# Corv/CUDA-GMM-MPI

Measured on NVIDIA H100. Metric: EM iterations/sec at N=10M D=24 K=64; E-step HBM GB/s vs roofline, higher is better.
Workload: dtype f32

## Files before the change

cuda-gmm-mpi_b200/csrc/kernels_tc.cu:

```cuda
#include <cuda.h>
#include <cudaTypedefs.h>
#include <cuda_fp16.h>
#if defined(__F16C__) && defined(__AVX__)
#include <immintrin.h>
#endif
#include <cuda_runtime.h>

#include <cmath>
#include <cstdio>
#include <cstdlib>
#include <cstring>
#include <string>
#include <type_traits>
#include <vector>

#include "host_math.h"
#include "kernels_tc.cuh"
#include "mstep_rows.h"
#include "tc_ptx.cuh"

namespace gmm {

using namespace ptx;

// ... 269 lines not shown
        auto add_to_racc = [&](float (&acc)[HPC][NCL / 2]) {
#pragma unroll
            for (int c = 0; c < 2; c++) {
#pragma unroll
                for (int j = 0; j < 16; j++) {
                    const int q = 16 * c + j;
                    racc[q * C::NCT] += acc[q / (NCL / 2)][q % (NCL / 2)];
                }
                asm volatile("" ::: "memory");
            }
        };
        uint32_t fh[2][2][4], fl[2][2][4];
        float2 za[4];
        int held = -1;
        auto group = [&](int i, auto hc, uint32_t (&gh)[2][4], uint32_t (&gl)[2][4]) {
            constexpr int h = decltype(hc)::value;
            const int rs = i % kNRAW, rph = (i / kNRAW) & 1;
            const int os = i % kNST, oph = (i / kNST) & 1;
            const uint32_t zst = zs0 + rs * C::RAWX;
            const uint32_t gam = smem_u32(smem + C::OFF_G + os * C::G_STAGE);
            const bool new1 = chain_starts(i, mt), new2 = chain2_starts(i, mt);
            if constexpr (h == 0) {
                mbar_wait_parked(&raw_full[rs], rph, 100);
                load_row(zst + fa, za);
            }
            float2 zb0[4], zb1[4];
            load_row(zst + fb[2 * h], zb0);
            load_row(zst + fb[2 * h + 1], zb1);
            build_half(za, zb0, zb1, mg[2 * h], mg[2 * h + 1], gh, gl);
            if constexpr (h == 0) mbar_wait_parked(&op_full[os], oph, 100);
            wgmma_fence();
            issue_half<NCL>(ex[h], rm[h], gh, gl, gam, new1, new2);
            wgmma_commit();
            if constexpr (h == HPC - 1) {
                __syncwarp();
                if (lane == 0) mbar_arrive(&raw_empty[rs]);
            }
            wgmma_wait<1>();
            if constexpr (h == 0) {
                __syncwarp();
                if (lane == 0 && held >= 0) mbar_arrive(&op_empty[held]);
            }
            if constexpr (h == HPC - 1) {
                held = os;
                if (chain_ends(i, mt, nsub)) {
                    wgmma_wait<0>();
                    __syncwarp();
                    if (lane == 0) mbar_arrive(&op_empty[os]);
                    held = -1;
#if GMM_MSTEP_CUT != 3
                    add_to_racc(ex);
                    if (chain2_ends(i, mt, nsub)) add_to_racc(rm);
#endif
                }
            }
        };
        using H0 = std::integral_constant<int, 0>;
        using H1 = std::integral_constant<int, 1>;
        if constexpr (HPC == 2) {
            for (int i = 0; i < nsub; i++) {
                group(i, H0{}, fh[0], fl[0]);
                group(i, H1{}, fh[1], fl[1]);
            }
        } else {
            int i = 0;
            for (; i + 1 < nsub; i += 2) {
                group(i, H0{}, fh[0], fl[0]);
                group(i + 1, H0{}, fh[1], fl[1]);
            }
            if (i < nsub) group(i, H0{}, fh[0], fl[0]);
        }
        wgmma_wait<0>();
#if GMM_MSTEP_CUT == 3
#pragma unroll
        for (int h = 0; h < HPC; h++)
#pragma unroll
            for (int j = 0; j < NCL / 2; j++) ex[h][j] += rm[h][j];
        add_to_racc(ex);
#endif
        const int nranges = gridDim.x * HPC / 2;
#pragma unroll
        for (int h = 0; h < HPC; h++)
#pragma unroll
            for (int j = 0; j < NCL / 2; j += 2) {
                const int q = h * (NCL / 2) + j;
                const int row = ((hx & 1) + h) * 64 + wq * 16 + gid + 8 * ((j >> 1) & 1);
                const int col = (j >> 2) * 8 + 2 * qd;
                const int ty = blockIdx.y * (NCL / kNCL) + col / kNCL;
                float* dst = scratch + ((((size_t)ty * nranges + range) * C::MT + mt) * 128 + row) * kNCL + col % kNCL;
                *reinterpret_cast<float2*>(dst) = make_float2(racc[q * C::NCT], racc[(q + 1) * C::NCT]);
            }
    }
}

__global__ void standardise_soa_kernel(const float* __restrict__ xs, float* __restrict__ zs, size_t pitch, int n, int D,
                                       const float* __restrict__ shift_f, const float* __restrict__ inv_scale_f) {
    const int d = blockIdx.y;
    const float s = shift_f[d], isc = inv_scale_f[d];
    const float* x = xs + (size_t)d * pitch;
    float* z = zs + (size_t)d * pitch;
    for (long long e = (long long)blockIdx.x * blockDim.x + threadIdx.x; e < n; e += (long long)gridDim.x * blockDim.x)
        z[e] = __fmul_rn(__fsub_rn(x[e], s), isc);
}

__global__ void __launch_bounds__(256)
mstep_tc_finalize_kernel(const float* __restrict__ scratch, int ncta_x, int MT, int K, int F, const int3* __restrict__ rowmap,
                         const double* __restrict__ scale, double* __restrict__ stats, double wscale) {
    constexpr int NQ = 256 / kNCL;
    __shared__ double part[NQ][kNCL];
    const int3 rm = rowmap[blockIdx.x];
    if (rm.x < 0) return;
    const int mt = blockIdx.x / 128, row = blockIdx.x % 128;
    const int col = threadIdx.x & (kNCL - 1), q = threadIdx.x / kNCL;
    double fac = wscale / (double)kGammaScale;
    if (rm.y >= 0) fac *= scale[rm.y];
    if (rm.z >= 0) fac *= scale[rm.z];
    for (int ty = 0; ty * kNCL < K; ty++) {
        double s = 0;
        for (int cx = q; cx < ncta_x; cx += NQ)
            s += (double)scratch[(((size_t)(ty * ncta_x + cx) * MT + mt) * 128 + row) * kNCL + col];
        part[q][col] = s;
        __syncthreads();
        const int k = ty * kNCL + col;
        if (q == 0 && k < K) {
            double t = 0;
#pragma unroll
            for (int u = 0; u < NQ; u++) t += part[u][col];
            stats[(size_t)k * F + rm.x] += t * fac;
        }
        __syncthreads();
    }
}


template <int D> struct ECfg {
    static_assert(D % 8 == 0, "tensor E-step: D must be a multiple of 8");
    static constexpr int CP = D / 8;
    static constexpr int NLO = (CP + 1 + 1) / 2 * 2;
    static constexpr int NCHKB = CP + NLO;
    static constexpr int GB = 16;
    static constexpr int N = GB * 8;
    static constexpr int MAXSG = 64 / GB;
    static constexpr int B_BLOCK = NCHKB * N * 16;
    static constexpr int B_SG = CP * B_BLOCK;
    static constexpr int OFF_B = 0;
    static constexpr int OFF_CK = OFF_B + MAXSG * B_SG;
    static constexpr int OFF_SH = OFF_CK + 512;
    static constexpr int OFF_BAR = OFF_SH + 256;
    static constexpr int SMEM_BYTES = OFF_BAR + 64;
    static constexpr int NWG = 2;
    static constexpr int THREADS = 128 * NWG;
};

#ifndef GMM_ESTEP_CUT
#define GMM_ESTEP_CUT 0
#endif

template <int D>
__device__ __forceinline__ void tc_stage_operand(uint8_t* smem, const uint8_t* __restrict__ b_img, const float* __restrict__ ck,
                                                 const float* __restrict__ shift_f, const float* __restrict__ inv_scale_f, int NSG) {
    using C = ECfg<D>;
    uint64_t* b_full = reinterpret_cast<uint64_t*>(smem + C::OFF_BAR);
    float* ck_s = reinterpret_cast<float*>(smem + C::OFF_CK);
    float* sh_s = reinterpret_cast<float*>(smem + C::OFF_SH);
    if (threadIdx.x == 0) { mbar_init(b_full, 1); fence_mbar_init(); }
    if (threadIdx.x < 64) { ck_s[threadIdx.x] = ck[threadIdx.x] * 1.4426950408889634f; ck_s[64 + threadIdx.x] = ck[64 + threadIdx.x]; }
    if (threadIdx.x < D) { sh_s[threadIdx.x] = shift_f[threadIdx.x]; sh_s[32 + threadIdx.x] = inv_scale_f[threadIdx.x]; }
    __syncthreads();
    if (threadIdx.x == 0) {
        mbar_arrive_expect_tx(b_full, (uint32_t)NSG * C::B_SG);
        for (int g = 0; g < NSG * C::CP; g++) tma_load_1d(smem + C::OFF_B + g * C::B_BLOCK, b_img + (size_t)g * C::B_BLOCK, C::B_BLOCK, b_full);
    }
}

template <int D>
__device__ __forceinline__ void tc_split_rows(const float2 (&xa)[D / 8], const float2 (&xb)[D / 8], const float* sh_s, const float* isc_s,
                                              int qd, uint32_t (&zh)[D / 8][2], uint32_t (&zl)[D / 8][2]) {
#pragma unroll
    for (int j = 0; j < D / 8; j++) {
        const float s0 = sh_s[8 * j + 2 * qd], s1 = sh_s[8 * j + 2 * qd + 1];
        const float i0 = isc_s[8 * j + 2 * qd], i1 = isc_s[8 * j + 2 * qd + 1];
#pragma unroll
        for (int r = 0; r < 2; r++) {
            const float2 x = r ? xb[j] : xa[j];
            const float z0 = __fmul_rn(__fsub_rn(x.x, s0), i0), z1 = __fmul_rn(__fsub_rn(x.y, s1), i1);
            const __half2 h = __floats2half2_rn(z0, z1);
            const float2 f = __half22float2(h);
            zh[j][r] = *reinterpret_cast<const uint32_t*>(&h);
            zl[j][r] = pack_half2(z0 - f.x, z1 - f.y);
        }
    }
}

template <int D>
__device__ __forceinline__ void tc_issue_group(float (&acc)[32], const uint32_t (&zh)[D / 8][2], const uint32_t (&zl)[D / 8][2],
                                               uint32_t bsg, int c, int h, uint32_t ones) {
    using C = ECfg<D>;
    constexpr int CP = C::CP;
    constexpr uint32_t CH = C::N * 16;
    const uint32_t bb = bsg + (uint32_t)c * C::B_BLOCK + (uint32_t)h * (CH / 2);
    wgmma_fence();
#pragma unroll
    for (int j = c; j < CP; j++)
        wgmma_m64n64k16_rs(acc, zh[j][0], zh[j][1], zh[j][0], zh[j][1], make_smem_desc(bb + j * CH, CP * CH, 128), j > c);
#pragma unroll
    for (int p = c; p < CP + 1; p += 2) {
        const int x = p, y = p + 1;
        if (y <= CP) {
            const uint32_t yc = y < CP ? (uint32_t)y : 2u * CP;
            const uint32_t a2 = y < CP ? zl[y < CP ? y : 0][0] : ones, a3 = y < CP ? zl[y < CP ? y : 0][1] : ones;
            wgmma_m64n64k16_rs(acc, zl[x][0], zl[x][1], a2, a3, make_smem_desc(bb + x * CH, (yc - x) * CH, 128), true);
        } else {
            wgmma_m64n64k16_rs(acc, 0u, 0u, ones, ones, make_smem_desc(bb + c * CH, (2 * CP - c) * CH, 128), true);
        }
    }
}

template <int D, int NSG>
__device__ __forceinline__ void tc_tile_logits(const uint32_t (&zh)[D / 8][2], const uint32_t (&zl)[D / 8][2], uint32_t bsm,
                                               const float* ck_s, int qd, uint32_t ones, float (&lg)[ECfg<D>::MAXSG][8]) {
    using C = ECfg<D>;
    constexpr int CP = C::CP;
    float acc[2][32];
    tc_issue_group<D>(acc[0], zh, zl, bsm, 0, 0, ones);
    wgmma_commit();
#pragma unroll
    for (int sg = 0; sg < C::MAXSG; sg++) {
        if (sg >= NSG) {
#pragma unroll
            for (int u = 0; u < 8; u++) lg[sg][u] = -INFINITY;
            continue;
        }
        const uint32_t bsg = bsm + (uint32_t)sg * C::B_SG;
        float sq[32];
#pragma unroll
        for (int u = 0; u < 32; u++) sq[u] = 0.f;
#pragma unroll
        for (int c = 0; c < CP; c++) {
#pragma unroll
            for (int h = 0; h < 2; h++) {
                if (sg + 1 == NSG && c + 1 == CP && h == 1) {
                    wgmma_wait<0>();
                } else {
                    if (h == 0) tc_issue_group<D>(acc[1], zh, zl, bsg, c, 1, ones);
                    else if (c + 1 < CP) tc_issue_group<D>(acc[0], zh, zl, bsg, c + 1, 0, ones);
                    else tc_issue_group<D>(acc[0], zh, zl, bsg + C::B_SG, 0, 0, ones);
                    wgmma_commit();
                    wgmma_wait<1>();
                }
                wgmma_pin(acc[h]);
                const float(&a)[32] = acc[h];
#if GMM_ESTEP_CUT == 1
                sq[0] += a[0];
#else
#pragma unroll
                for (int i = 0; i < 8; i++) {
                    float& s0 = sq[16 * h + 2 * i];
                    float& s1 = sq[16 * h + 2 * i + 1];
                    s0 = fmaf(a[4 * i], a[4 * i], fmaf(a[4 * i + 1], a[4 * i + 1], s0));
                    s1 = fmaf(a[4 * i + 2], a[4 * i + 2], fmaf(a[4 * i + 3], a[4 * i + 3], s1));
                }
#endif
            }
        }
#if GMM_ESTEP_CUT == 1
        for (int u = 0; u < 8; u++) lg[sg][u] = sq[0];
        continue;
#endif
        float w[16];
        const bool b1 = qd & 1, b2 = (qd >> 1) & 1;
#pragma unroll
        for (int u = 0; u < 16; u++) {
            const float send = b1 ? sq[u] : sq[16 + u], keep = b1 ? sq[16 + u] : sq[u];
            w[u] = keep + __shfl_xor_sync(0xffffffffu, send, 1);
        }
#pragma unroll
        for (int u = 0; u < 8; u++) {
            const float send = b2 ? w[u] : w[8 + u], keep = b2 ? w[8 + u] : w[u];
            const float qv = keep + __shfl_xor_sync(0xffffffffu, send, 2);
            const int k = sg * C::GB + 8 * (qd & 1) + 4 * (qd >> 1) + (u >> 1);
            lg[sg][u] = fmaf(ck_s[64 + k], qv, ck_s[k]);
        }
    }
}

template <int D, int NSG, bool WT = false>
__global__ void __launch_bounds__(ECfg<D>::THREADS, 1)
estep_tc_kernel(const float* __restrict__ x_aos, const uint8_t* __restrict__ b_img, const float* __restrict__ ck,
                const float* __restrict__ shift_f, const float* __restrict__ inv_scale_f, float* __restrict__ memb,
                size_t pitch, int n, int K, double* __restrict__ ll_out, int mode, const float* den_in, float* den_out,
                const float* __restrict__ wts) {
    using C = ECfg<D>;
    constexpr int CP = C::CP;
    extern __shared__ __align__(1024) uint8_t smem[];
    uint64_t* b_full = reinterpret_cast<uint64_t*>(smem + C::OFF_BAR);
    float* ck_s = reinterpret_cast<float*>(smem + C::OFF_CK);
    float* sh_s = reinterpret_cast<float*>(smem + C::OFF_SH);
    float* isc_s = sh_s + 32;

    const int wg = threadIdx.x >> 7, warp = (threadIdx.x >> 5) & 3, lane = threadIdx.x & 31;
    const int gid = lane >> 2, qd = lane & 3;
    const int ntiles = (n + 63) / 64;

    tc_stage_operand<D>(smem, b_img, ck, shift_f, inv_scale_f, NSG);

    const int r0 = warp * 16 + gid;
    float2 xa[CP], xb[CP];
    auto load_rows = [&](int t) {
        const long long e0 = (long long)t * 64 + r0, e1 = e0 + 8;
#pragma unroll
        for (int j = 0; j < CP; j++) {
            xa[j] = e0 < n ? __ldg(reinterpret_cast<const float2*>(x_aos + (size_t)e0 * D + 8 * j + 2 * qd)) : make_float2(0.f, 0.f);
            xb[j] = e1 < n ? __ldg(reinterpret_cast<const float2*>(x_aos + (size_t)e1 * D + 8 * j + 2 * qd)) : make_float2(0.f, 0.f);
        }
    };
    const int stride = (int)gridDim.x * C::NWG;
    int t = (int)blockIdx.x * C::NWG + wg;
    if (t < ntiles) load_rows(t);
    const uint32_t ones = qd == 0 ? 0x3C003C00u : 0u;
    const uint32_t bsm = smem_u32(smem + C::OFF_B);
    double ll_acc = 0.0;
    constexpr float kLn2 = 0.6931471805599453f;
    mbar_wait(b_full, 0);

    for (; t < ntiles; t += stride) {
        uint32_t zh[CP][2], zl[CP][2];
        tc_split_rows<D>(xa, xb, sh_s, isc_s, qd, zh, zl);
        const long long e0 = (long long)t * 64 + r0, e1 = e0 + 8;
        if (t + stride < ntiles) load_rows(t + stride);

        float lg[C::MAXSG][8];
        tc_tile_logits<D, NSG>(zh, zl, bsm, ck_s, qd, ones, lg);
#if GMM_ESTEP_CUT == 1
        for (int sg = 0; sg < C::MAXSG; sg++) ll_acc += (double)lg[sg][0];
        continue;
#endif
        float mx[2] = {-INFINITY, -INFINITY};
#pragma unroll
        for (int sg = 0; sg < C::MAXSG; sg++)
#pragma unroll
            for (int u = 0; u < 8; u++) mx[u & 1] = fmaxf(mx[u & 1], lg[sg][u]);
#pragma unroll
        for (int r = 0; r < 2; r++) {
            mx[r] = fmaxf(mx[r], __shfl_xor_sync(0xffffffffu, mx[r], 1));
            mx[r] = fmaxf(mx[r], __shfl_xor_sync(0xffffffffu, mx[r], 2));
        }
        float scale[2] = {1.f, 1.f};
        const long long er[2] = {e0, e1};
        if (mode == 3) {
            float d2[2];
#pragma unroll
            for (int r = 0; r < 2; r++) d2[r] = er[r] < n ? den_in[er[r]] * 1.4426950408889634f : 0.f;
#pragma unroll
            for (int sg = 0; sg < C::MAXSG; sg++)
#pragma unroll
                for (int u = 0; u < 8; u++) lg[sg][u] = ex2_approx(lg[sg][u] - d2[u & 1]);
        } else {
            float sm[2] = {0.f, 0.f};
#pragma unroll
            for (int sg = 0; sg < C::MAXSG; sg++)
#pragma unroll
                for (int u = 0; u < 8; u++) { lg[sg][u] = ex2_approx(lg[sg][u] - mx[u & 1]); sm[u & 1] += lg[sg][u]; }
            float dx[2];
#pragma unroll
            for (int r = 0; r < 2; r++) {
                sm[r] += __shfl_xor_sync(0xffffffffu, sm[r], 1);
                sm[r] += __shfl_xor_sync(0xffffffffu, sm[r], 2);
                dx[r] = (mode != 0 && den_in != nullptr && er[r] < n) ? den_in[er[r]] : 0.f;
            }
            __syncwarp();
#pragma unroll
            for (int r = 0; r < 2; r++) {
                float denom = fmaf(mx[r], kLn2, logf(sm[r]));
                scale[r] = 1.0f / sm[r];
                if (mode != 0 && er[r] < n) {
                    if (den_in != nullptr) {
                        const float g = fmaxf(denom, dx[r]);
                        const float tot = g + logf(__expf(denom - g) + __expf(dx[r] - g));
                        scale[r] *= __expf(denom - tot);
                        denom = tot;
                    }
                    if (qd == 0) den_out[er[r]] = denom;
                }
                if constexpr (WT) {
                    if (qd == 0 && er[r] < n && (mode == 0 || mode == 2)) ll_acc += (double)wts[er[r]] * (double)denom;
                } else {
                    if (qd == 0 && er[r] < n && (mode == 0 || mode == 2)) ll_acc += (double)denom;
                }
            }
        }
        if (mode != 1 && GMM_ESTEP_CUT != 2) {
#pragma unroll
            for (int sg = 0; sg < C::MAXSG; sg++) {
#pragma unroll
                for (int u = 0; u < 8; u++) {
                    const int k = sg * C::GB + 8 * (qd & 1) + 4 * (qd >> 1) + (u >> 1);
                    const long long e = er[u & 1];
                    if (sg < NSG && (k & ~7) < K && e < n) memb[(size_t)k * pitch + e] = lg[sg][u] * scale[u & 1];
                }
            }
        }
    }
    if (mode == 0 || mode == 2) {
        ll_acc = ll_acc + __shfl_down_sync(0xffffffffu, ll_acc, 16);
        ll_acc = ll_acc + __shfl_down_sync(0xffffffffu, ll_acc, 8);
        ll_acc = ll_acc + __shfl_down_sync(0xffffffffu, ll_acc, 4);
        ll_acc = ll_acc + __shfl_down_sync(0xffffffffu, ll_acc, 2);
        ll_acc = ll_acc + __shfl_down_sync(0xffffffffu, ll_acc, 1);
        if (lane == 0) atomicAdd(ll_out, ll_acc);
    }
}

template <int D, int NSG>
__global__ void __launch_bounds__(ECfg<D>::THREADS, 1)
score_tc_kernel(const float* __restrict__ x_aos, const uint8_t* __restrict__ b_img, const float* __restrict__ ck,
                const float* __restrict__ shift_f, const float* __restrict__ inv_scale_f, int n, int K, int kbase,
                int pass, int last, float* run_den, float* run_bl, int* run_bk, int* __restrict__ labels,
                float* __restrict__ max_resp, float* __restrict__ logp, double* __restrict__ ll_out, int* __restrict__ flag) {
    using C = ECfg<D>;
    constexpr int CP = C::CP;
    extern __shared__ __align__(1024) uint8_t smem[];
    uint64_t* b_full = reinterpret_cast<uint64_t*>(smem + C::OFF_BAR);
    const float* ck_s = reinterpret_cast<const float*>(smem + C::OFF_CK);
    const float* sh_s = reinterpret_cast<const float*>(smem + C::OFF_SH);
    const float* isc_s = sh_s + 32;

    const int wg = threadIdx.x >> 7, warp = (threadIdx.x >> 5) & 3, lane = threadIdx.x & 31;
    const int gid = lane >> 2, qd = lane & 3;
    const int ntiles = (n + 63) / 64;
    tc_stage_operand<D>(smem, b_img, ck, shift_f, inv_scale_f, NSG);

    const int r0 = warp * 16 + gid;
    float2 xa[CP], xb[CP];
    auto load_rows = [&](int t) {
        const long long e0 = (long long)t * 64 + r0, e1 = e0 + 8;
#pragma unroll
        for (int j = 0; j < CP; j++) {
            xa[j] = e0 < n ? __ldg(reinterpret_cast<const float2*>(x_aos + (size_t)e0 * D + 8 * j + 2 * qd)) : make_float2(0.f, 0.f);
            xb[j] = e1 < n ? __ldg(reinterpret_cast<const float2*>(x_aos + (size_t)e1 * D + 8 * j + 2 * qd)) : make_float2(0.f, 0.f);
        }
    };
    const int stride = (int)gridDim.x * C::NWG;
    int t = (int)blockIdx.x * C::NWG + wg;
    if (t < ntiles) load_rows(t);
    const uint32_t ones = qd == 0 ? 0x3C003C00u : 0u;
    const uint32_t bsm = smem_u32(smem + C::OFF_B);
    double ll_acc = 0.0;
    constexpr float kLn2 = 0.6931471805599453f, kLog2e = 1.4426950408889634f;
    bool out_of_range = false;
    mbar_wait(b_full, 0);

    for (; t < ntiles; t += stride) {
        const long long e0 = (long long)t * 64 + r0, e1 = e0 + 8;
#pragma unroll
        for (int j = 0; j < CP; j++)
#pragma unroll
            for (int r = 0; r < 2; r++) {
                const float2 x = r ? xb[j] : xa[j];
                const float z0 = __fmul_rn(__fsub_rn(x.x, sh_s[8 * j + 2 * qd]), isc_s[8 * j + 2 * qd]);
                const float z1 = __fmul_rn(__fsub_rn(x.y, sh_s[8 * j + 2 * qd + 1]), isc_s[8 * j + 2 * qd + 1]);
                out_of_range |= (r ? e1 : e0) < n && (!(fabsf(z0) <= 16384.0f) || !(fabsf(z1) <= 16384.0f));
            }
        uint32_t zh[CP][2], zl[CP][2];
        tc_split_rows<D>(xa, xb, sh_s, isc_s, qd, zh, zl);
        if (t + stride < ntiles) load_rows(t + stride);

        float lg[C::MAXSG][8];
        tc_tile_logits<D, NSG>(zh, zl, bsm, ck_s, qd, ones, lg);

        float mx[2] = {-INFINITY, -INFINITY}, bl[2] = {-INFINITY, -INFINITY};
        int bk[2] = {-1, -1};
#pragma unroll
        for (int sg = 0; sg < C::MAXSG; sg++)
#pragma unroll
            for (int u = 0; u < 8; u++) {
                const float l = lg[sg][u];
                const int k = sg * C::GB + 8 * (qd & 1) + 4 * (qd >> 1) + (u >> 1);
                mx[u & 1] = fmaxf(mx[u & 1], l);
                if (k < K && (l > bl[u & 1] || (bk[u & 1] < 0 && l == l))) { bl[u & 1] = l; bk[u & 1] = kbase + k; }
            }
#pragma unroll
        for (int r = 0; r < 2; r++) {
            mx[r] = fmaxf(mx[r], __shfl_xor_sync(0xffffffffu, mx[r], 1));
            mx[r] = fmaxf(mx[r], __shfl_xor_sync(0xffffffffu, mx[r], 2));
#pragma unroll
            for (int o = 1; o <= 2; o <<= 1) {
                const float ov = __shfl_xor_sync(0xffffffffu, bl[r], o);
                const int ok = __shfl_xor_sync(0xffffffffu, bk[r], o);
                if (ok >= 0 && (bk[r] < 0 || ov > bl[r] || (ov == bl[r] && ok < bk[r]))) { bl[r] = ov; bk[r] = ok; }
            }
        }
        float sm[2] = {0.f, 0.f};
#pragma unroll
        for (int sg = 0; sg < C::MAXSG; sg++)
#pragma unroll
            for (int u = 0; u < 8; u++) sm[u & 1] += ex2_approx(lg[sg][u] - mx[u & 1]);
        const long long er[2] = {e0, e1};
        float dx[2] = {0.f, 0.f}, pbl[2] = {0.f, 0.f};
        int pbk[2] = {-1, -1};
#pragma unroll
        for (int r = 0; r < 2; r++) {
            sm[r] += __shfl_xor_sync(0xffffffffu, sm[r], 1);
            sm[r] += __shfl_xor_sync(0xffffffffu, sm[r], 2);
            if (pass > 0 && er[r] < n) { dx[r] = run_den[er[r]]; pbl[r] = run_bl[er[r]]; pbk[r] = run_bk[er[r]]; }
        }
        __syncwarp();
#pragma unroll
        for (int r = 0; r < 2; r++) {
            float denom = fmaf(mx[r], kLn2, logf(sm[r]));
            float mr = ex2_approx(bl[r] - mx[r]) * (1.0f / sm[r]);
            if (pass > 0) {
                const float g = fmaxf(denom, dx[r]);
                const float tot = g + logf(__expf(denom - g) + __expf(dx[r] - g));
                if (bk[r] >= 0 && (pbk[r] < 0 || bl[r] > pbl[r])) {
                    const float sc = (1.0f / sm[r]) * __expf(denom - tot);
                    mr = ex2_approx(bl[r] - mx[r]) * sc;
                } else {
                    bl[r] = pbl[r]; bk[r] = pbk[r];
                    mr = ex2_approx(bl[r] - __fmul_rn(tot, kLog2e));
                }
                denom = tot;
            }
            if (qd == 0 && er[r] < n) {
                if (last) {
                    labels[er[r]] = bk[r];
                    max_resp[er[r]] = bk[r] >= 0 ? mr : __int_as_float(0x7fc00000);
                    logp[er[r]] = denom;
                    ll_acc += (double)denom;
                } else {
                    run_den[er[r]] = denom; run_bl[er[r]] = bl[r]; run_bk[er[r]] = bk[r];
                }
            }
        }
    }
    if (__any_sync(0xffffffffu, out_of_range) && lane == 0) *flag = 1;
    if (last) {
        ll_acc = ll_acc + __shfl_down_sync(0xffffffffu, ll_acc, 16);
        ll_acc = ll_acc + __shfl_down_sync(0xffffffffu, ll_acc, 8);
        ll_acc = ll_acc + __shfl_down_sync(0xffffffffu, ll_acc, 4);
        ll_acc = ll_acc + __shfl_down_sync(0xffffffffu, ll_acc, 2);
        ll_acc = ll_acc + __shfl_down_sync(0xffffffffu, ll_acc, 1);
        if (lane == 0) atomicAdd(ll_out, ll_acc);
    }
}

struct TcState {
    const float* d_x = nullptr;
    const float* d_x_soa = nullptr;
    float* d_z_soa = nullptr;
    float* d_memb = nullptr;
    size_t memb_pitch = 0;
    int n = 0, D = 0, Kmax = 0, num_sms = 132;
    CUtensorMap tm_x{}, tm_g{};
    bool maps_ok = false;
    float* d_shift_f = nullptr;
    float* d_inv_scale_f = nullptr;
    double* d_scale = nullptr;
    float* d_scratch = nullptr;
    size_t scratch_floats = 0;
    bool have_shift = false;
    bool mstep_ready = false;
    float zmax[GMM_MAX_DIMENSIONS] = {0};
// ... 449 lines not shown
        } else if (tid == j) {
            sU[j][j] = piv;
        }
        __syncthreads();
    }
    if (!ok) {
        if (tid == 0) { atomicCAS(&bad[0], -1, iter); atomicMax(&bad[1], 1); }
        return;
    }
    FIN_STAMP(3);
    if (tid < D) {
        const int j = tid;
        for (int i = D - 1; i > j; i--) sW[i][j] = 0.0;
        sW[j][j] = 1.0 / sU[j][j];
        for (int i = j - 1; i >= 0; i--) {
            double v = 0.0;
            for (int m = i + 1; m <= j; m++) v = __dsub_rn(v, __dmul_rn(sU[i][m], sW[m][j]));
            sW[i][j] = v / sU[i][i];
        }
    }
    if (tid == T - 1) {
        double sum = 0.0;
        for (int kk = 0; kk < K; kk++) sum += (double)sN[kk];
        ssumN = sum;
    }
    __syncthreads();
    FIN_STAMP(4);
    const float pik = Nf < 0.5f ? 1e-10f : (float)((double)Nf / ssumN);
    {
        float* Ri = set + pset_off_Rinv(Kmax, D) + (size_t)k * D * D;
        for (int idx = tid; idx < D * D; idx += T) {
            const int i = idx / D, j = idx % D;
            if (j < i) continue;
            double v = 0.0;
#pragma unroll 4
            for (int m = 0; m <= i; m++) v = __dadd_rn(v, __dmul_rn(sW[m][i], sW[m][j]));
            Ri[i * D + j] = (float)v; Ri[j * D + i] = (float)v;
        }
    }
    FIN_STAMP(5);
    float amax = 0.f;
    for (int idx = tid; idx < D * D; idx += T) {
        const int d = idx / D, j = idx % D;
        const float w = (j >= d) ? (float)(sW[d][j] * sscale[j]) : 0.f;
        swr[d][j] = w;
        amax = fmaxf(amax, fabsf(w));
    }
    if (tid >= 64 && tid < 64 + D) {
        const int d = tid - 64;
        double v = 0.0;
#pragma unroll 4
        for (int j = d; j < D; j++) v = fma(-sW[d][j], sdm[j], v);
        svd[d] = v;
        amax = fmaxf(amax, (float)fabs(v));
    }
    if (tid == 32) {
        double ld = 0.0;
        for (int j = D - 1; j >= 0; j--) ld += log(sU[j][j]);
        sredd[0] = ld;
    }
#pragma unroll
    for (int o = 16; o > 0; o >>= 1) amax = fmaxf(amax, __shfl_xor_sync(0xffffffffu, amax, o));
    if ((tid & 31) == 0) sredf[tid >> 5] = amax;
    __syncthreads();
    FIN_STAMP(6);
    const double ld = sredd[0];
    const float cst = (float)(-D * 0.5 * log(2.0 * 3.1415926535897931) - 0.5 * (2.0 * ld));
    if (tid == 0) { set[k] = Nf; set[Kmax + k] = pik; set[2 * (size_t)Kmax + k] = cst; }
    amax = 0.f;
#pragma unroll
    for (int w = 0; w < NW; w++) amax = fmaxf(amax, sredf[w]);
    if (!isfinite(amax)) {
        if (tid == 0) { atomicCAS(&bad[0], -1, iter); atomicMax(&bad[1], 2); }
        return;
    }
    int e2 = amax > 0.f ? 12 - ilogbf(amax) : 0;
    e2 = e2 > 40 ? 40 : (e2 < -40 ? -40 : e2);
    for (int idx = tid; idx < D * C::CP; idx += T) {
        const int d = idx / C::CP, c = idx % C::CP;
        uint32_t hi[4], lo[4];
#pragma unroll
        for (int e = 0; e < 4; e++) {
            const float w0 = ldexpf(swr[d][8 * c + 2 * e], e2), w1 = ldexpf(swr[d][8 * c + 2 * e + 1], e2);
            const __half2 h = __floats2half2_rn(w0, w1);
            const float2 hf = __half22float2(h);
            hi[e] = *reinterpret_cast<const uint32_t*>(&h);
            lo[e] = pack_half2(w0 - hf.x, w1 - hf.y);
        }
        *reinterpret_cast<uint4*>(rowp(d, c)) = make_uint4(hi[0], hi[1], hi[2], hi[3]);
        *reinterpret_cast<uint4*>(rowp(d, C::CP + c)) = make_uint4(lo[0], lo[1], lo[2], lo[3]);
    }
    if (tid >= 128 && tid < 128 + D) {
        const int d = tid - 128;
        const double vs = ldexp(svd[d], e2);
        const float vf = (float)vs;
        if (!(fabsf(vf) < 6.0e4f)) atomicMax(&sbad, 2);
        const __half vh = __float2half_rn(vf);
        const __half vl = __float2half_rn((float)(vs - (double)__half2float(vh)));
        const uint32_t p = (uint32_t)__half_as_ushort(vh) | ((uint32_t)__half_as_ushort(vl) << 16);
        *reinterpret_cast<uint4*>(rowp(d, 2 * C::CP)) = make_uint4(p, 0u, 0u, 0u);
        if (C::NCHKB > 2 * C::CP + 1) *reinterpret_cast<uint4*>(rowp(d, 2 * C::CP + 1)) = make_uint4(0u, 0u, 0u, 0u);
    }
    if (tid == 0) {
        ckp[0] = cst + (float)log((double)pik);
        ckp[64] = (float)ldexp(-0.5 * 1.4426950408889634, -2 * e2);
    }
    __syncthreads();
    FIN_STAMP(7);
#ifdef GMM_FIN_PROF
    if (k == 0 && tid == 0)
        printf("fin phases (cycles): stage %lld  means+R %lld  cholesky %lld  inverse %lld  Rinv %lld  rows+v+log %lld  operand %lld\n",
               fin_t[1] - fin_t[0], fin_t[2] - fin_t[1], fin_t[3] - fin_t[2], fin_t[4] - fin_t[3], fin_t[5] - fin_t[4], fin_t[6] - fin_t[5], fin_t[7] - fin_t[6]);
#endif
    if (tid == 0 && sbad) { atomicCAS(&bad[0], -1, iter); atomicMax(&bad[1], sbad); }
}

size_t tc_param_set_floats(int Kmax, int D) { return (size_t)Kmax * (3 + (size_t)D + 2 * (size_t)D * D); }
size_t tc_param_set_off(int Kmax, int D, int which) {
    switch (which) {
        case 0: return 0;
        case 1: return (size_t)Kmax;
        case 2: return 2 * (size_t)Kmax;
        case 3: return pset_off_means(Kmax);
        case 4: return pset_off_R(Kmax, D);
        default: return pset_off_Rinv(Kmax, D);
    }
}
bool tc_finalize_supported(const TcState* t, int K) {
    return t && t->emap_ok && t->have_shift && tc_estep_supported(t->D, K) && tc_estep_range_ok(t);
}
int tc_launch_finalize(TcState* t, int K, const double* d_stats, const float* d_avgvar, float* d_set, double* d_ll, int* d_bad, int iter,
                       int fault_iter, cudaStream_t stream) {
    if (!tc_finalize_supported(t, K)) return fail(GMM_ERR_STATE, "device-side finalisation not available for this state");
    const int kp = tc_params_padded(t, K);
    const int grid = ((K + 63) / 64) * 64;
#define GMM_FIN(d) finalize_params_kernel<d><<<grid, FinCfg<d>::T, 0, stream>>>(d_stats, d_avgvar, t->d_shift_f, t->d_scale, d_set, t->Kmax, K, kp, \
                                                                     t->d_bimg, t->d_ck, d_ll, d_bad, iter, fault_iter)
    switch (t->D) {
        case 8: GMM_FIN(8); break;
        case 16: GMM_FIN(16); break;
        case 24: GMM_FIN(24); break;
        default: return fail(GMM_ERR_ARG, "device-side finalisation: unsupported D");
    }
#undef GMM_FIN
    TC_CUDA_TRY(cudaGetLastError());
    t->e_NG = (K + 15) / 16;
    return GMM_OK;
}

template <int D>
static int launch_estep_d(TcState* t, int K, const float* x, int n, float* memb, size_t pitch, float* den, double* d_ll, const float* w,
                          cudaStream_t stream) {
    using C = ECfg<D>;
    static_assert(C::SMEM_BYTES <= 232448, "shared memory budget");
    using KernFn = void (*)(const float*, const uint8_t*, const float*, const float*, const float*, float*, size_t, int, int, double*, int,
                            const float*, float*, const float*);
    static const KernFn kern0[C::MAXSG] = {estep_tc_kernel<D, 1>, estep_tc_kernel<D, 2>, estep_tc_kernel<D, 3>, estep_tc_kernel<D, 4>};
    static const KernFn kern1[C::MAXSG] = {estep_tc_kernel<D, 1, true>, estep_tc_kernel<D, 2, true>, estep_tc_kernel<D, 3, true>,
                                           estep_tc_kernel<D, 4, true>};
    static_assert(C::MAXSG == 4, "one kernel instance per supergroup count");
    if (!t->attr_estep) {
        for (auto* k : kern0) TC_CUDA_TRY(cudaFuncSetAttribute(k, cudaFuncAttributeMaxDynamicSharedMemorySize, C::SMEM_BYTES));
        for (auto* k : kern1) TC_CUDA_TRY(cudaFuncSetAttribute(k, cudaFuncAttributeMaxDynamicSharedMemorySize, C::SMEM_BYTES));
        t->attr_estep = true;
    }
    const KernFn* kern = w ? kern1 : kern0;
    const int ntiles = (n + 127) / 128;
    int grid = t->num_sms;
    if (grid > ntiles) grid = ntiles;
    if (grid < 1) grid = 1;
    const int NP = (K + 63) / 64;
    if (NP > 1 && !den) return fail(GMM_ERR_STATE, "tensor E-step: context was created for at most 64 clusters");
    auto launch = [&](int p, int mode, const float* den_in, float* den_out) {
        const int Kp = K - 64 * p < 64 ? K - 64 * p : 64;
        kern[(Kp + C::GB - 1) / C::GB - 1]<<<grid, C::THREADS, C::SMEM_BYTES, stream>>>(
            x, t->d_bimg + (size_t)p * C::MAXSG * C::B_SG, t->d_ck + 128 * p, t->d_shift_f, t->d_inv_scale_f,
            memb + (size_t)(64 * p) * pitch, pitch, n, Kp, d_ll, mode, den_in, den_out, w);
        return cudaGetLastError();
    };
    if (NP == 1) TC_CUDA_TRY(launch(0, 0, nullptr, nullptr));
    else {
        for (int p = 0; p + 1 < NP; p++) TC_CUDA_TRY(launch(p, 1, p ? den : nullptr, den));
        TC_CUDA_TRY(launch(NP - 1, 2, den, den));
        for (int p = 0; p + 1 < NP; p++) TC_CUDA_TRY(launch(p, 3, den, nullptr));
    }
    return GMM_OK;
}

static int launch_estep_any(TcState* t, int K, const float* x, int n, float* memb, size_t pitch, float* den, double* d_ll, const float* w,
                            cudaStream_t stream) {
    if (!t || !t->emap_ok) return fail(GMM_ERR_STATE, "tensor E-step not initialised for this shape");
    switch (t->D) {
        case 8: return launch_estep_d<8>(t, K, x, n, memb, pitch, den, d_ll, w, stream);
        case 16: return launch_estep_d<16>(t, K, x, n, memb, pitch, den, d_ll, w, stream);
        case 24: return launch_estep_d<24>(t, K, x, n, memb, pitch, den, d_ll, w, stream);
        default: return fail(GMM_ERR_ARG, "tensor E-step: unsupported D");
    }
}

int tc_launch_estep(TcState* t, int K, double* d_ll, cudaStream_t stream, const float* d_w) {
    if (!t) return fail(GMM_ERR_STATE, "tensor E-step not initialised for this shape");
    return launch_estep_any(t, K, t->d_x, t->n, t->d_memb, t->memb_pitch, t->d_den, d_ll, d_w, stream);
}

int tc_launch_estep_on(TcState* t, int K, const float* d_x_aos, int n, float* d_memb, size_t pitch, float* d_den, double* d_ll,
                       cudaStream_t stream) {
    if (n <= 0) return GMM_OK;
    return launch_estep_any(t, K, d_x_aos, n, d_memb, pitch, d_den, d_ll, nullptr, stream);
}

template <int D>
static int launch_score_d(TcState* t, int K, const TcScoreIo& io, cudaStream_t stream) {
    using C = ECfg<D>;
    static void (*const kern[C::MAXSG])(const float*, const uint8_t*, const float*, const float*, const float*, int, int, int, int, int,
                                        float*, float*, int*, int*, float*, float*, double*, int*) = {
        score_tc_kernel<D, 1>, score_tc_kernel<D, 2>, score_tc_kernel<D, 3>, score_tc_kernel<D, 4>};
    static_assert(C::MAXSG == 4, "one kernel instance per supergroup count");
    if (!t->attr_score) {
        for (auto* k : kern) TC_CUDA_TRY(cudaFuncSetAttribute(k, cudaFuncAttributeMaxDynamicSharedMemorySize, C::SMEM_BYTES));
        t->attr_score = true;
    }
    const int ntiles = (io.n + 127) / 128;
    int grid = t->num_sms;
    if (grid > ntiles) grid = ntiles;
    if (grid < 1) grid = 1;
    const int NP = (K + 63) / 64;
    if (NP > 1 && !(io.run_den && io.run_bl && io.run_bk)) return fail(GMM_ERR_STATE, "tensor scoring: no running state for K > 64");
    for (int p = 0; p < NP; p++) {
        const int Kp = K - 64 * p < 64 ? K - 64 * p : 64;
        kern[(Kp + C::GB - 1) / C::GB - 1]<<<grid, C::THREADS, C::SMEM_BYTES, stream>>>(
            io.x, t->d_bimg + (size_t)p * C::MAXSG * C::B_SG, t->d_ck + 128 * p, t->d_shift_f, t->d_inv_scale_f, io.n, Kp, 64 * p, p, p + 1 == NP, io.run_den, io.run_bl, io.run_bk, io.labels, io.max_resp, io.logp, io.ll,
            io.flag);
        TC_CUDA_TRY(cudaGetLastError());
    }
    return GMM_OK;
}

int tc_launch_score(TcState* t, int K, const TcScoreIo& io, cudaStream_t stream) {
    if (!t || !t->emap_ok) return fail(GMM_ERR_STATE, "tensor scoring not initialised for this shape");
    if (io.n <= 0) return GMM_OK;
    switch (t->D) {
        case 8: return launch_score_d<8>(t, K, io, stream);
        case 16: return launch_score_d<16>(t, K, io, stream);
        case 24: return launch_score_d<24>(t, K, io, stream);
        default: return fail(GMM_ERR_ARG, "tensor scoring: unsupported D");
    }
}

template <int D>
static int launch_mstep_d(TcState* t, int K, const CUtensorMap& tm_x, const CUtensorMap& tm_g, int n, double* d_stats, const float* w,
                          double wscale, cudaStream_t stream) {
    using C32 = MCfg<D, 32>;
    using C64 = MCfg<D, 64>;
    static_assert(C32::SMEM_BYTES <= 232448 && C64::SMEM_BYTES <= 232448, "shared memory budget");
    if (!t->attr_mstep) {
        TC_CUDA_TRY(cudaFuncSetAttribute(mstep_tc_kernel<D, 32>, cudaFuncAttributeMaxDynamicSharedMemorySize, C32::SMEM_BYTES));
        TC_CUDA_TRY(cudaFuncSetAttribute(mstep_tc_kernel<D, 64>, cudaFuncAttributeMaxDynamicSharedMemorySize, C64::SMEM_BYTES));
        TC_CUDA_TRY(cudaFuncSetAttribute(mstep_tc_kernel<D, 32, true>, cudaFuncAttributeMaxDynamicSharedMemorySize, C32::SMEM_BYTES));
        TC_CUDA_TRY(cudaFuncSetAttribute(mstep_tc_kernel<D, 64, true>, cudaFuncAttributeMaxDynamicSharedMemorySize, C64::SMEM_BYTES));
        t->attr_mstep = true;
    }
    const float w_max = (float)wscale, w_inv = (float)(1.0 / wscale);
    int gx = t->num_sms;
    int per = (n + gx - 1) / gx;
    per = (per + kTE - 1) / kTE * kTE;
    gx = (n + per - 1) / per;
    const bool pair = K > 32;
    const int ncl = pair ? 64 : 32;
    const int gy = (K + ncl - 1) / ncl;
    if ((size_t)gx * gy * (ncl / kNCL) * C32::MT * 128 * kNCL > t->scratch_floats) return fail(GMM_ERR_STATE, "tensor M-step scratch too small");
    const dim3 grid(pair ? 2 * gx : gx, gy);
    if (pair) {
        if (w) mstep_tc_kernel<D, 64, true><<<grid, C64::THREADS, C64::SMEM_BYTES, stream>>>(tm_x, tm_g, n, K, t->d_scratch, per, t->magic, t->d_opmap, w, w_max, w_inv);
        else mstep_tc_kernel<D, 64><<<grid, C64::THREADS, C64::SMEM_BYTES, stream>>>(tm_x, tm_g, n, K, t->d_scratch, per, t->magic, t->d_opmap, nullptr, 1.0f, 1.0f);
    } else {
        if (w) mstep_tc_kernel<D, 32, true><<<grid, C32::THREADS, C32::SMEM_BYTES, stream>>>(tm_x, tm_g, n, K, t->d_scratch, per, t->magic, t->d_opmap, w, w_max, w_inv);
        else mstep_tc_kernel<D, 32><<<grid, C32::THREADS, C32::SMEM_BYTES, stream>>>(tm_x, tm_g, n, K, t->d_scratch, per, t->magic, t->d_opmap, nullptr, 1.0f, 1.0f);
    }
    TC_CUDA_TRY(cudaGetLastError());
    mstep_tc_finalize_kernel<<<C32::MT * 128, 256, 0, stream>>>(t->d_scratch, gx, C32::MT, K, C32::F, t->d_rowmap, t->d_scale, d_stats,
                                                                w ? wscale : 1.0);
    TC_CUDA_TRY(cudaGetLastError());
    return GMM_OK;
}

static int launch_mstep_any(TcState* t, int K, const CUtensorMap& tm_x, const CUtensorMap& tm_g, int n, double* d_stats, const float* w,
                            double wscale, cudaStream_t stream) {
    if (!t || !t->maps_ok) return fail(GMM_ERR_STATE, "tensor-core M-step not initialised for this shape");
    if (!t->have_shift) return fail(GMM_ERR_STATE, "tensor-core M-step needs gmm_seed (shift/scale) first");
    if (!t->mstep_ready) return fail(GMM_ERR_STATE, "tensor-core M-step: the data range exceeds the fixed-point operand budget");
    switch (t->D) {
        case 4: return launch_mstep_d<4>(t, K, tm_x, tm_g, n, d_stats, w, wscale, stream);
        case 8: return launch_mstep_d<8>(t, K, tm_x, tm_g, n, d_stats, w, wscale, stream);
        case 12: return launch_mstep_d<12>(t, K, tm_x, tm_g, n, d_stats, w, wscale, stream);
        case 16: return launch_mstep_d<16>(t, K, tm_x, tm_g, n, d_stats, w, wscale, stream);
        case 20: return launch_mstep_d<20>(t, K, tm_x, tm_g, n, d_stats, w, wscale, stream);
        case 24: return launch_mstep_d<24>(t, K, tm_x, tm_g, n, d_stats, w, wscale, stream);
        default: return fail(GMM_ERR_ARG, "tensor-core M-step: unsupported D");
    }
}

int tc_launch_mstep(TcState* t, int K, double* d_stats, cudaStream_t stream, const float* d_w, double wscale) {
    if (!t) return fail(GMM_ERR_STATE, "tensor-core M-step not initialised for this shape");
    return launch_mstep_any(t, K, t->tm_x, t->tm_g, t->n, d_stats, d_w, wscale, stream);
}

int tc_launch_mstep_on(TcState* t, int K, const float* d_z, const float* d_memb, size_t pitch, int n, double* d_stats, cudaStream_t stream) {
    if (n <= 0) return GMM_OK;
    if (!t || !t->maps_ok) return fail(GMM_ERR_STATE, "tensor-core M-step not initialised for this shape");
    if (t->cmap_z != d_z || t->cmap_g != d_memb || t->cmap_pitch != pitch || t->cmap_n != n) {
        t->cmap_n = -1;
        if (int rc = make_map_2d(&t->tm_cx, d_z, (uint64_t)n, (uint64_t)t->D, (uint64_t)pitch * 4, kTE, (uint32_t)t->D, true)) return rc;
        if (int rc = make_map_2d(&t->tm_cg, d_memb, (uint64_t)n, (uint64_t)t->Kmax, (uint64_t)pitch * 4, kTE, kNCL, true)) return rc;
        t->cmap_z = d_z; t->cmap_g = d_memb; t->cmap_pitch = pitch; t->cmap_n = n;
    }
    return launch_mstep_any(t, K, t->tm_cx, t->tm_cg, n, d_stats, nullptr, 1.0, stream);
}

const float* tc_shift_f(const TcState* t) { return t && t->have_shift ? t->d_shift_f : nullptr; }
const float* tc_inv_scale_f(const TcState* t) { return t && t->have_shift ? t->d_inv_scale_f : nullptr; }
float tc_mstep_zbound(const TcState* t) {
    float zb = 0.f;
    if (t)
        for (int d = 0; d < t->D; d++) zb = std::fmax(zb, t->zmax[d]);
    return zb;
}

}
// ... 1 lines not shown
```

Baseline: 136.1.

## Split E-step into warp-specialized MMA producer and softmax epilogue consumer warpgroups

For D>8 the E-step kernel now runs two MMA warpgroups that compute logits into a triple-buffered swizzled shared-memory slot ring, and two epilogue warpgroups that do the log-sum-exp, normalization and coalesced float4 stores of memberships. The two sides hand off through full/empty mbarriers, and registers are rebalanced with setmaxnreg. The aim is to overlap tensor-core work with the exp-heavy, store-bound epilogue so that HBM writes stay saturated. The cost is extra shared-memory round trips, more synchronization and tighter register budgets.

```diff
diff --git a/cuda-gmm-mpi_b200/csrc/kernels_tc.cu b/cuda-gmm-mpi_b200/csrc/kernels_tc.cu
--- a/cuda-gmm-mpi_b200/csrc/kernels_tc.cu
+++ b/cuda-gmm-mpi_b200/csrc/kernels_tc.cu
@@ -445,6 +445,36 @@
     static constexpr int THREADS = 128 * NWG;
 };
 
+template <int D> struct EsCfg {
+    using E = ECfg<D>;
+    static constexpr bool SPLIT = D > 8;
+    static constexpr int NMMA = 2;
+    static constexpr int THREADS = SPLIT ? 128 * 2 * NMMA : E::THREADS;
+    static constexpr int NSLOT = 3;
+    static constexpr int SLOT = 64 * 64 * 4;
+    static constexpr int OFF_SLOT = (E::SMEM_BYTES + 127) / 128 * 128;
+    static constexpr int OFF_STAT = OFF_SLOT + NSLOT * SLOT;
+    static constexpr int OFF_EBAR = OFF_STAT + NSLOT * 2 * 64 * 4;
+    static constexpr int SMEM_BYTES = SPLIT ? OFF_EBAR + 4 * NSLOT * 8 : E::SMEM_BYTES;
+    static constexpr int REG_LAUNCH = 65536 / (128 * 2 * NMMA) / 8 * 8;
+    static constexpr int REG_MMA = 184;
+    static constexpr int REG_EPI = 72;
+    static_assert(128 * NMMA * (REG_MMA + REG_EPI) <= 128 * 2 * NMMA * REG_LAUNCH, "register pools");
+    static_assert(SMEM_BYTES <= 232448, "shared memory budget");
+};
+
+__device__ __forceinline__ uint32_t slot_swz(int e) { return (uint32_t)(((e & 1) << 2 | (e & 2)) ^ ((e >> 2) & 7)); }
+
+__device__ __forceinline__ void sts_f4(uint32_t addr, float a, float b, float c, float d) {
+    asm volatile("st.shared.v4.f32 [%0], {%1, %2, %3, %4};" ::"r"(addr), "f"(a), "f"(b), "f"(c), "f"(d) : "memory");
+}
+__device__ __forceinline__ float4 lds_f4(uint32_t addr) {
+    float4 v;
+    asm volatile("ld.shared.v4.f32 {%0, %1, %2, %3}, [%4];" : "=f"(v.x), "=f"(v.y), "=f"(v.z), "=f"(v.w) : "r"(addr) : "memory");
+    return v;
+}
+__device__ __forceinline__ void epi_bar(int id) { asm volatile("bar.sync %0, 128;" ::"r"(id) : "memory"); }
+
 #ifndef GMM_ESTEP_CUT
 #define GMM_ESTEP_CUT 0
 #endif
@@ -577,9 +607,71 @@
     }
 }
 
-template <int D, int NSG, bool WT = false>
-__global__ void __launch_bounds__(ECfg<D>::THREADS, 1)
-estep_tc_kernel(const float* __restrict__ x_aos, const uint8_t* __restrict__ b_img, const float* __restrict__ ck,
+template <int D, int NSG>
+__device__ __forceinline__ void estep_tile_logits(const uint32_t (&zh)[D / 8][2], const uint32_t (&zl)[D / 8][2], uint32_t bsm,
+                                                  const float* ck_s, int qd, uint32_t ones, uint32_t slot, int r0, float& cut_sum) {
+    using C = ECfg<D>;
+    constexpr int CP = C::CP, NG = NSG * CP * 2;
+    float acc[2][32];
+    tc_issue_group<D>(acc[0], zh, zl, bsm, 0, 0, ones);
+    wgmma_commit();
+    const uint32_t cq = 2 * (qd & 1) + (qd >> 1);
+    const uint32_t row0 = slot + (uint32_t)r0 * 256, row1 = row0 + 8 * 256;
+    const uint32_t sw0 = slot_swz(r0), sw1 = slot_swz(r0 + 8);
+    float sq[32];
+#pragma unroll
+    for (int g = 0; g < NG; g++) {
+        const int sg = g / (2 * CP), c = (g / 2) % CP, h = g & 1;
+        if (c == 0 && h == 0) {
+#pragma unroll
+            for (int u = 0; u < 32; u++) sq[u] = 0.f;
+        }
+        if (g + 1 < NG) {
+            const int gn = g + 1;
+            tc_issue_group<D>(acc[gn & 1], zh, zl, bsm + (uint32_t)(gn / (2 * CP)) * C::B_SG, (gn / 2) % CP, gn & 1, ones);
+            wgmma_commit();
+            wgmma_wait<1>();
+        } else {
+            wgmma_wait<0>();
+        }
+        wgmma_pin(acc[g & 1]);
+        const float(&a)[32] = acc[g & 1];
+#if GMM_ESTEP_CUT == 1
+        cut_sum += a[0];
+#else
+#pragma unroll
+        for (int i = 0; i < 8; i++) {
+            float& s0 = sq[16 * h + 2 * i];
+            float& s1 = sq[16 * h + 2 * i + 1];
+            s0 = fmaf(a[4 * i], a[4 * i], fmaf(a[4 * i + 1], a[4 * i + 1], s0));
+            s1 = fmaf(a[4 * i + 2], a[4 * i + 2], fmaf(a[4 * i + 3], a[4 * i + 3], s1));
+        }
+        if (c == CP - 1 && h == 1) {
+            float w[16];
+            const bool b1 = qd & 1, b2 = (qd >> 1) & 1;
+#pragma unroll
+            for (int u = 0; u < 16; u++) {
+                const float send = b1 ? sq[u] : sq[16 + u], keep = b1 ? sq[16 + u] : sq[u];
+                w[u] = keep + __shfl_xor_sync(0xffffffffu, send, 1);
+            }
+            float l[8];
+#pragma unroll
+            for (int u = 0; u < 8; u++) {
+                const float send = b2 ? w[u] : w[8 + u], keep = b2 ? w[8 + u] : w[u];
+                const float qv = keep + __shfl_xor_sync(0xffffffffu, send, 2);
+                const int k = sg * C::GB + 8 * (qd & 1) + 4 * (qd >> 1) + (u >> 1);
+                l[u] = fmaf(ck_s[64 + k], qv, ck_s[k]);
+            }
+            const uint32_t ch = 4 * (uint32_t)sg + cq;
+            sts_f4(row0 + ((ch ^ sw0) << 4), l[0], l[2], l[4], l[6]);
+            sts_f4(row1 + ((ch ^ sw1) << 4), l[1], l[3], l[5], l[7]);
+        }
+#endif
+    }
+}
+
+template <int D, int NSG, bool WT>
+__device__ __forceinline__ void estep_fused(const float* __restrict__ x_aos, const uint8_t* __restrict__ b_img, const float* __restrict__ ck,
                 const float* __restrict__ shift_f, const float* __restrict__ inv_scale_f, float* __restrict__ memb,
                 size_t pitch, int n, int K, double* __restrict__ ll_out, int mode, const float* den_in, float* den_out,
                 const float* __restrict__ wts) {
@@ -701,6 +793,182 @@
         ll_acc = ll_acc + __shfl_down_sync(0xffffffffu, ll_acc, 2);
         ll_acc = ll_acc + __shfl_down_sync(0xffffffffu, ll_acc, 1);
         if (lane == 0) atomicAdd(ll_out, ll_acc);
+    }
+}
+
+template <int D, int NSG, bool WT = false>
+__global__ void __launch_bounds__(EsCfg<D>::THREADS, 1)
+estep_tc_kernel(const float* __restrict__ x_aos, const uint8_t* __restrict__ b_img, const float* __restrict__ ck,
+                const float* __restrict__ shift_f, const float* __restrict__ inv_scale_f, float* __restrict__ memb,
+                size_t pitch, int n, int K, double* __restrict__ ll_out, int mode, const float* den_in, float* den_out,
+                const float* __restrict__ wts) {
+    if constexpr (!EsCfg<D>::SPLIT) {
+        estep_fused<D, NSG, WT>(x_aos, b_img, ck, shift_f, inv_scale_f, memb, pitch, n, K, ll_out, mode, den_in, den_out, wts);
+        return;
+    } else {
+    using E = ECfg<D>;
+    using C = EsCfg<D>;
+    constexpr int CP = E::CP;
+    extern __shared__ __align__(1024) uint8_t smem[];
+    uint64_t* b_full = reinterpret_cast<uint64_t*>(smem + E::OFF_BAR);
+    uint64_t* full = reinterpret_cast<uint64_t*>(smem + C::OFF_EBAR);
+    uint64_t* empty = full + 2 * C::NSLOT;
+    const float* ck_s = reinterpret_cast<const float*>(smem + E::OFF_CK);
+    const float* sh_s = reinterpret_cast<const float*>(smem + E::OFF_SH);
+    const float* isc_s = sh_s + 32;
+    const uint32_t slots = smem_u32(smem + C::OFF_SLOT);
+
+    const int wg = threadIdx.x >> 7, warp = (threadIdx.x >> 5) & 3, lane = threadIdx.x & 31;
+    const int ntiles = (n + 63) / 64;
+    const int stride = (int)gridDim.x * C::NMMA;
+    if (threadIdx.x == 0) {
+        for (int b = 0; b < 2 * C::NSLOT; b++) { mbar_init(&full[b], 128); mbar_init(&empty[b], 128); }
+    }
+    tc_stage_operand<D>(smem, b_img, ck, shift_f, inv_scale_f, NSG);
+
+    if (wg < C::NMMA) {
+        set_regs<C::REG_MMA, C::REG_LAUNCH>();
+        const int gid = lane >> 2, qd = lane & 3;
+        const int r0 = warp * 16 + gid;
+        float2 xa[CP], xb[CP];
+        auto load_rows = [&](int t) {
+            const long long e0 = (long long)t * 64 + r0, e1 = e0 + 8;
+#pragma unroll
+            for (int j = 0; j < CP; j++) {
+                xa[j] = e0 < n ? __ldg(reinterpret_cast<const float2*>(x_aos + (size_t)e0 * D + 8 * j + 2 * qd)) : make_float2(0.f, 0.f);
+                xb[j] = e1 < n ? __ldg(reinterpret_cast<const float2*>(x_aos + (size_t)e1 * D + 8 * j + 2 * qd)) : make_float2(0.f, 0.f);
+            }
+        };
+        int t = (int)blockIdx.x * C::NMMA + wg;
+        if (t < ntiles) load_rows(t);
+        const uint32_t ones = qd == 0 ? 0x3C003C00u : 0u;
+        const uint32_t bsm = smem_u32(smem + E::OFF_B);
+        float cut_sum = 0.f;
+        mbar_wait(b_full, 0);
+        for (int i = wg; t < ntiles; t += stride, i += C::NMMA) {
+            uint32_t zh[CP][2], zl[CP][2];
+            tc_split_rows<D>(xa, xb, sh_s, isc_s, qd, zh, zl);
+            if (t + stride < ntiles) load_rows(t + stride);
+            const int s = i % C::NSLOT, u = i / C::NSLOT;
+#if GMM_ESTEP_CUT != 1
+            if (u > 0) mbar_wait(&empty[2 * s + ((u - 1) & 1)], ((u - 1) >> 1) & 1);
+#endif
+            estep_tile_logits<D, NSG>(zh, zl, bsm, ck_s, qd, ones, slots + (uint32_t)s * C::SLOT, r0, cut_sum);
+#if GMM_ESTEP_CUT != 1
+            mbar_arrive(&full[2 * s + (u & 1)]);
+#endif
+        }
+        if (GMM_ESTEP_CUT == 1 && cut_sum == -1.f) atomicAdd(ll_out, 0.0);
+        return;
+    }
+
+    set_regs<C::REG_EPI, C::REG_LAUNCH>();
+    if (GMM_ESTEP_CUT == 1) return;
+    const int ew = wg - C::NMMA, et = threadIdx.x & 127;
+    const int ev = et >> 1, hh = et & 1;
+    const uint32_t evrow = (uint32_t)ev * 256, evswz = slot_swz(ev);
+    float* stat = reinterpret_cast<float*>(smem + C::OFF_STAT);
+    const uint32_t stat_u = smem_u32(stat);
+    double ll_acc = 0.0;
+    constexpr float kLn2 = 0.6931471805599453f, kLog2e = 1.4426950408889634f;
+    for (int i = ew;; i += C::NMMA) {
+        const int t = (int)blockIdx.x * C::NMMA + i % C::NMMA + (i / C::NMMA) * stride;
+        if (t >= ntiles) break;
+        const int s = i % C::NSLOT;
+        const uint32_t slot = slots + (uint32_t)s * C::SLOT;
+        const int u = i / C::NSLOT, sb2 = 2 * s + (u & 1);
+        mbar_wait(&full[sb2], (u >> 1) & 1);
+        const long long e = (long long)t * 64 + ev;
+        float sub, scl = 1.f, dep = 0.f;
+        if (mode == 3) {
+            sub = e < n ? den_in[e] * kLog2e : 0.f;
+        } else {
+            float mx = -INFINITY;
+#pragma unroll
+            for (int sg = 0; sg < NSG; sg++)
+#pragma unroll
+                for (int j = 0; j < 2; j++) {
+                    const float4 v = lds_f4(slot + evrow + (((uint32_t)(4 * sg + 2 * j + hh) ^ evswz) << 4));
+                    mx = fmaxf(fmaxf(mx, v.x), fmaxf(fmaxf(v.y, v.z), v.w));
+                }
+            mx = fmaxf(mx, __shfl_xor_sync(0xffffffffu, mx, 1));
+            float p0 = 0.f, p1 = 0.f;
+#pragma unroll
+            for (int sg = 0; sg < NSG; sg++) {
+                const float4 v0 = lds_f4(slot + evrow + (((uint32_t)(4 * sg + hh) ^ evswz) << 4));
+                const float4 v1 = lds_f4(slot + evrow + (((uint32_t)(4 * sg + 2 + hh) ^ evswz) << 4));
+                p0 += ex2_approx(v0.x - mx); p0 += ex2_approx(v0.y - mx); p0 += ex2_approx(v0.z - mx); p0 += ex2_approx(v0.w - mx);
+                p1 += ex2_approx(v1.x - mx); p1 += ex2_approx(v1.y - mx); p1 += ex2_approx(v1.z - mx); p1 += ex2_approx(v1.w - mx);
+            }
+            const float a = p0 + p1;
+            const float S = a + __shfl_xor_sync(0xffffffffu, a, 1);
+            sub = mx;
+            dep = S;
+            if (hh == 0) {
+                float denom = fmaf(mx, kLn2, logf(S));
+                scl = 1.0f / S;
+                if (mode != 0 && e < n) {
+                    if (den_in != nullptr) {
+                        const float dx = den_in[e];
+                        const float g = fmaxf(denom, dx);
+                        const float tot = g + logf(__expf(denom - g) + __expf(dx - g));
+                        scl *= __expf(denom - tot);
+                        denom = tot;
+                    }
+                    den_out[e] = denom;
+                }
+                if constexpr (WT) {
+                    if (e < n && (mode == 0 || mode == 2)) ll_acc += (double)wts[e] * (double)denom;
+                } else {
+                    if (e < n && (mode == 0 || mode == 2)) ll_acc += (double)denom;
+                }
+            }
+        }
+        if (mode == 1 || GMM_ESTEP_CUT == 2) {
+            mbar_arrive_after(&empty[sb2], dep);
+            continue;
+        }
+        if (hh == 0) { stat[s * 128 + ev] = sub; stat[s * 128 + 64 + ev] = scl; }
+        epi_bar(1 + ew);
+#pragma unroll 1
+        for (int j = 0; j < 2; j++) {
+            const int b = et + 128 * j, c = b >> 4, a = b & 15;
+            if (c >= 4 * NSG || (4 * c & ~7) >= K) continue;
+            float4 v[4];
+#pragma unroll
+            for (int m = 0; m < 4; m++) v[m] = lds_f4(slot + (uint32_t)(4 * a + m) * 256 + (((uint32_t)c ^ slot_swz(4 * a + m)) << 4));
+            const float4 sb = lds_f4(stat_u + (uint32_t)s * 512 + 16 * a), sc = lds_f4(stat_u + (uint32_t)s * 512 + 256 + 16 * a);
+            dep += (v[0].x + v[1].x) + (v[2].x + v[3].x);
+            const long long e0 = (long long)t * 64 + 4 * a;
+            float* dst = memb + (size_t)(4 * c) * pitch + e0;
+#pragma unroll
+            for (int q = 0; q < 4; q++) {
+                const float l0 = q == 0 ? v[0].x : q == 1 ? v[0].y : q == 2 ? v[0].z : v[0].w;
+                const float l1 = q == 0 ? v[1].x : q == 1 ? v[1].y : q == 2 ? v[1].z : v[1].w;
+                const float l2 = q == 0 ? v[2].x : q == 1 ? v[2].y : q == 2 ? v[2].z : v[2].w;
+                const float l3 = q == 0 ? v[3].x : q == 1 ? v[3].y : q == 2 ? v[3].z : v[3].w;
+                const float4 gm = make_float4(ex2_approx(l0 - sb.x) * sc.x, ex2_approx(l1 - sb.y) * sc.y, ex2_approx(l2 - sb.z) * sc.z,
+                                              ex2_approx(l3 - sb.w) * sc.w);
+                float* row = dst + (size_t)q * pitch;
+                if (e0 + 3 < n) {
+                    *reinterpret_cast<float4*>(row) = gm;
+                } else {
+                    if (e0 < n) row[0] = gm.x;
+                    if (e0 + 1 < n) row[1] = gm.y;
+                    if (e0 + 2 < n) row[2] = gm.z;
+                }
+            }
+        }
+        mbar_arrive_after(&empty[sb2], dep);
+    }
+    if (mode == 0 || mode == 2) {
+        ll_acc = ll_acc + __shfl_down_sync(0xffffffffu, ll_acc, 16);
+        ll_acc = ll_acc + __shfl_down_sync(0xffffffffu, ll_acc, 8);
+        ll_acc = ll_acc + __shfl_down_sync(0xffffffffu, ll_acc, 4);
+        ll_acc = ll_acc + __shfl_down_sync(0xffffffffu, ll_acc, 2);
+        ll_acc = ll_acc + __shfl_down_sync(0xffffffffu, ll_acc, 1);
+        if (lane == 0) atomicAdd(ll_out, ll_acc);
+    }
     }
 }
 
@@ -1456,7 +1724,7 @@
 static int launch_estep_d(TcState* t, int K, const float* x, int n, float* memb, size_t pitch, float* den, double* d_ll, const float* w,
                           cudaStream_t stream) {
     using C = ECfg<D>;
-    static_assert(C::SMEM_BYTES <= 232448, "shared memory budget");
+    using L = EsCfg<D>;
     using KernFn = void (*)(const float*, const uint8_t*, const float*, const float*, const float*, float*, size_t, int, int, double*, int,
                             const float*, float*, const float*);
     static const KernFn kern0[C::MAXSG] = {estep_tc_kernel<D, 1>, estep_tc_kernel<D, 2>, estep_tc_kernel<D, 3>, estep_tc_kernel<D, 4>};
@@ -1464,8 +1732,8 @@
                                            estep_tc_kernel<D, 4, true>};
     static_assert(C::MAXSG == 4, "one kernel instance per supergroup count");
     if (!t->attr_estep) {
-        for (auto* k : kern0) TC_CUDA_TRY(cudaFuncSetAttribute(k, cudaFuncAttributeMaxDynamicSharedMemorySize, C::SMEM_BYTES));
-        for (auto* k : kern1) TC_CUDA_TRY(cudaFuncSetAttribute(k, cudaFuncAttributeMaxDynamicSharedMemorySize, C::SMEM_BYTES));
+        for (auto* k : kern0) TC_CUDA_TRY(cudaFuncSetAttribute(k, cudaFuncAttributeMaxDynamicSharedMemorySize, L::SMEM_BYTES));
+        for (auto* k : kern1) TC_CUDA_TRY(cudaFuncSetAttribute(k, cudaFuncAttributeMaxDynamicSharedMemorySize, L::SMEM_BYTES));
         t->attr_estep = true;
     }
     const KernFn* kern = w ? kern1 : kern0;
@@ -1477,7 +1745,7 @@
     if (NP > 1 && !den) return fail(GMM_ERR_STATE, "tensor E-step: context was created for at most 64 clusters");
     auto launch = [&](int p, int mode, const float* den_in, float* den_out) {
         const int Kp = K - 64 * p < 64 ? K - 64 * p : 64;
-        kern[(Kp + C::GB - 1) / C::GB - 1]<<<grid, C::THREADS, C::SMEM_BYTES, stream>>>(
+        kern[(Kp + C::GB - 1) / C::GB - 1]<<<grid, L::THREADS, L::SMEM_BYTES, stream>>>(
             x, t->d_bimg + (size_t)p * C::MAXSG * C::B_SG, t->d_ck + 128 * p, t->d_shift_f, t->d_inv_scale_f,
             memb + (size_t)(64 * p) * pitch, pitch, n, Kp, d_ll, mode, den_in, den_out, w);
         return cudaGetLastError();
```

After: 141.3 (median of 6 runs). +3.8%, better.
